# NJUVISION/PCGCv1

Hardware: AMD Instinct MI355X
Metric: 64³ cubes/sec encode+decode (hyper/a6b3); bpp & D1-PSNR vs reference (higher is better)
Workload: dtype f32; 1 GPU; synthetic longdress_vox10-like cloud (seed 1300, 1024^3): 828225 points -> 205 cubes of 64^3, --mode=hyper --cube_size=64 --min_num=64, the hyper/a6b3 checkpoint trained with this repository's train_hyper step on seeded synthetic surfaces (checkpoints/hyper/a6.00b3.00, tools/train_ckpt.py; the cloud was held out), compress_hyper + decompress_hyper incl. host range coding; cubes_per_rank=205, stream_crc32=2267905730

## Files before the change

### pcgcv1_amd/csrc/vrn_row16.hip

```cpp
#include "row_common.h"

namespace pcgc {

constexpr int kW16 = 16;
constexpr int kRowQ16 = kW16 * 16;

__device__ __forceinline__ float rshr1(float v) {
  return __builtin_bit_cast(float, __builtin_amdgcn_update_dpp(0, __builtin_bit_cast(int, v), 0x111, 0xf, 0xf, true));
}
__device__ __forceinline__ float rshl1(float v) {
  return __builtin_bit_cast(float, __builtin_amdgcn_update_dpp(0, __builtin_bit_cast(int, v), 0x101, 0xf, 0xf, true));
}

template <int NQ>
__device__ __forceinline__ f32x4 load_vec(i32x4 rs, int lane_off, int lane_row, int p, int q, int a) {
  const bool ok = (unsigned)p < (unsigned)kW16 && (unsigned)(a + lane_row) < (unsigned)kW16;
  const int base = ((p * kW16 + a) * NQ + q) * kRowQ16;
  return raw_load4(rs, ok ? base + lane_off : kOOB, 0, 0);
}

struct Tile16 {
  int b, k, d0;
};
template <int LD>
__device__ __forceinline__ Tile16 wave_tile16() {
  int wv = __builtin_amdgcn_readfirstlane(blockIdx.x * 8 + (threadIdx.x >> 6));
  Tile16 t;
  t.k = wv % 4; wv /= 4;
  t.d0 = (wv % (kW16 / LD)) * LD; wv /= (kW16 / LD);
  t.b = wv;
  return t;
}

constexpr int kVrn64ImgA = 16 * 28 * 64, kVrn64ImgB = 8 * 27 * 64, kVrn64ImgC = 4 * 27 * 64;
constexpr int kVrn64ImageFloats = kVrn64ImgA + kVrn64ImgB + kVrn64ImgC;

struct Vrn64Args {
  const float* img = nullptr;
  const float* x;
  float* t12;
  float* out;
  const float *w11, *b11, *w21, *b21, *w12, *b12, *w22, *b22, *w23, *b23;
  int B;
};

template <int NCO, int NC, int W2 = -1>
__device__ __forceinline__ void vec_channels(f32x4 (&acc)[3][NCO], f32x4* acc2, const float (&W)[28], int c0, const f32x4 (&X)[3], bool v0,
                                             bool v1, bool v2) {
  float x0[NC][3], xm[NC][3], xp[NC][3];
#pragma unroll
  for (int c = 0; c < NC; ++c)
#pragma unroll
    for (int kh = 0; kh < 3; ++kh) { x0[c][kh] = comp(X[kh], c0 + c); xm[c][kh] = rshr1(x0[c][kh]); xp[c][kh] = rshl1(x0[c][kh]); }
  const bool vj[3] = {v0, v1, v2};
#pragma unroll
  for (int jj = 0; jj < 3; ++jj) {
    const int kd = 2 - jj;
    if (vj[jj]) {
#pragma unroll
      for (int c = 0; c < NC; ++c) {
#pragma unroll
        for (int kh = 0; kh < 3; ++kh)
#pragma unroll
          for (int kw = 0; kw < 3; ++kw) {
            const int t = (kd * 3 + kh) * 3 + kw;
            const float xv = kw == 0 ? xm[c][kh] : (kw == 1 ? x0[c][kh] : xp[c][kh]);
#pragma unroll
            for (int coq = 0; coq < NCO; ++coq) acc[jj][coq] = mfa((c0 + c) * 4 + coq, W[t], xv, acc[jj][coq]);
          }
        if constexpr (W2 >= 0) {
          if (jj == 1) {
#pragma unroll
            for (int coq = 0; coq < NCO; ++coq) acc2[coq] = mfa((c0 + c) * 4 + coq, W[W2], x0[c][1], acc2[coq]);
          }
        }
      }
    }
  }
}

constexpr int kA64Chunk = 28 * 64;

template <int LD, bool = true>
__global__ void __launch_bounds__(512, 2) vrn64a_row_kernel(Vrn64Args a) {
  constexpr int CH = kA64Chunk;
  __shared__ float wl[16 * CH];
  if (a.img) stage_image_t<16 * CH, 512>(wl, a.img);
  else
    for (int i = threadIdx.x; i < 16 * CH; i += 512) {
      const int q = i / CH, f = i - q * CH;
      wl[i] = f < 1728 ? a.w11[((f >> 6) * 64 + 4 * q + ((f >> 4) & 3)) * 16 + (f & 15)] : a.w21[(4 * q + ((f - 1728) >> 4)) * 16 + (f & 15)];
    }
  __syncthreads();
  const int lane = threadIdx.x & 63;
  const int lane_row = lane >> 4;
  const Tile16 tl = wave_tile16<LD>();
  if (tl.b >= a.B) return;
  const int r0 = 4 * tl.k, d0 = tl.d0;
  f32x4 bi[4], bi2[4];
#pragma unroll
  for (int q = 0; q < 4; ++q) {
    bi[q] = f32x4{a.b11[4 * q], a.b11[4 * q + 1], a.b11[4 * q + 2], a.b11[4 * q + 3]};
    bi2[q] = f32x4{a.b21[4 * q], a.b21[4 * q + 1], a.b21[4 * q + 2], a.b21[4 * q + 3]};
  }
  f32x4 acc[3][4], acc2[4];
#pragma unroll
  for (int j = 0; j < 3; ++j)
#pragma unroll
    for (int q = 0; q < 4; ++q) acc[j][q] = bi[q];
  const i32x4 rs = make_rsrc(a.x + (size_t)tl.b * kW16 * kW16 * kW16 * 64, kW16 * kW16 * kW16 * 64 * 4);
  const int lane_off = lane_row * (16 * kRowQ16) + (lane & 15) * 16;
  f32x4* tb = reinterpret_cast<f32x4*>(a.t12) + (size_t)tl.b * kW16 * kW16 * 8 * kW16 + lane_row * (8 * kW16) + (lane & 15);
  f32x4 XA[3], XB[3];
  auto load = [&](f32x4 (&X)[3], int p, int q) {
#pragma unroll
    for (int kh = 0; kh < 3; ++kh) X[kh] = load_vec<16>(rs, lane_off, lane_row, p, q, r0 + kh - 1);
  };
  auto fetch = [&](float (&W)[28], int q) {
#pragma unroll
    for (int v = 0; v < 28; ++v) W[v] = wl[q * CH + v * 64 + lane];
  };
  auto quad = [&](const f32x4 (&X)[3], const float (&W)[28], bool v0, bool v1, bool v2) {
    vec_channels<4, 4, 27>(acc, acc2, W, 0, X, v0, v1, v2);
  };
  float WA[28], WB[28];
  load(XA, d0 - 1, 0);
  fetch(WA, 0);
#pragma unroll 1
  for (int p = d0 - 1; p <= d0 + LD; ++p) {
    const bool pin = (unsigned)p < (unsigned)kW16;
    const bool v0 = pin && p - 1 >= d0, v1 = pin && p >= d0 && p < d0 + LD, v2 = pin && p + 1 < d0 + LD;
#pragma unroll
    for (int q = 0; q < 4; ++q) acc2[q] = bi2[q];
#pragma unroll 1
    for (int q = 0; q < 16; q += 2) {
      load(XB, p, q + 1);
      fetch(WB, q + 1);
      quad(XA, WA, v0, v1, v2);
      if (q + 2 < 16) load(XA, p, q + 2); else load(XA, p + 1, 0);
      fetch(WA, (q + 2) & 15);
      quad(XB, WB, v0, v1, v2);
    }
    if (v1) {
#pragma unroll
      for (int coq = 0; coq < 4; ++coq) tb[((size_t)(p * kW16 + r0) * 8 + 4 + coq) * kW16] = relu4(acc2[coq]);
    }
    if (p - 1 >= d0) {
#pragma unroll
      for (int coq = 0; coq < 4; ++coq) tb[((size_t)((p - 1) * kW16 + r0) * 8 + coq) * kW16] = relu4(acc[0][coq]);
    }
#pragma unroll
    for (int coq = 0; coq < 4; ++coq) { acc[0][coq] = acc[1][coq]; acc[1][coq] = acc[2][coq]; acc[2][coq] = bi[coq]; }
  }
}

template <int LD, bool = true>
__global__ void __launch_bounds__(512, 2) vrn64b_row_kernel(Vrn64Args a) {
  constexpr int CH = 27 * 64;
  __shared__ float wl[8 * CH];
  if (a.img) stage_image_t<8 * CH, 512>(wl, a.img + kVrn64ImgA);
  else
    for (int i = threadIdx.x; i < 8 * CH; i += 512) {
      const int qh = i / CH, f = i - qh * CH, q = qh >> 1, half = qh & 1;
      wl[i] = a.w12[((f >> 6) * 16 + 4 * q + ((f >> 4) & 3)) * 32 + 16 * half + (f & 15)];
    }
  __syncthreads();
  const int lane = threadIdx.x & 63;
  const int lane_row = lane >> 4;
  const Tile16 tl = wave_tile16<LD>();
  if (tl.b >= a.B) return;
  const int r0 = 4 * tl.k, d0 = tl.d0;
  f32x4 bi[8];
#pragma unroll
  for (int q = 0; q < 8; ++q) bi[q] = f32x4{a.b12[4 * q], a.b12[4 * q + 1], a.b12[4 * q + 2], a.b12[4 * q + 3]};
  f32x4 accL[3][4], accH[3][4];
#pragma unroll
  for (int j = 0; j < 3; ++j)
#pragma unroll
    for (int q = 0; q < 4; ++q) { accL[j][q] = bi[q]; accH[j][q] = bi[4 + q]; }
  const i32x4 rs = make_rsrc(a.t12 + (size_t)tl.b * kW16 * kW16 * kW16 * 32, kW16 * kW16 * kW16 * 32 * 4);
  const i32x4 rx = make_rsrc(a.x + (size_t)tl.b * kW16 * kW16 * kW16 * 64, kW16 * kW16 * kW16 * 64 * 4);
  const i32x4 ro = make_rsrc(a.out + (size_t)tl.b * kW16 * kW16 * kW16 * 64, kW16 * kW16 * kW16 * 64 * 4);
  const int lane_off = lane_row * (8 * kRowQ16) + (lane & 15) * 16;
  const int lane_off_x = lane_row * (16 * kRowQ16) + (lane & 15) * 16;
  f32x4 XA[3], XB[3];
  auto load = [&](f32x4 (&X)[3], int p, int q) {
#pragma unroll
    for (int kh = 0; kh < 3; ++kh) X[kh] = load_vec<8>(rs, lane_off, lane_row, p, q, r0 + kh - 1);
  };
  auto quad = [&](const f32x4 (&X)[3], int q, bool v0, bool v1, bool v2) {
    float W[28];
#pragma unroll
    for (int v = 0; v < 27; ++v) W[v] = wl[(2 * q) * CH + v * 64 + lane];
    vec_channels<4, 4>(accL, nullptr, W, 0, X, v0, v1, v2);
#pragma unroll
    for (int v = 0; v < 27; ++v) W[v] = wl[(2 * q + 1) * CH + v * 64 + lane];
    vec_channels<4, 4>(accH, nullptr, W, 0, X, v0, v1, v2);
  };
  load(XA, d0 - 1, 0);
#pragma unroll 1
  for (int p = d0 - 1; p <= d0 + LD; ++p) {
    const bool pin = (unsigned)p < (unsigned)kW16;
    const bool v0 = pin && p - 1 >= d0, v1 = pin && p >= d0 && p < d0 + LD, v2 = pin && p + 1 < d0 + LD;
    load(XB, p, 1);
    quad(XA, 0, v0, v1, v2);
    load(XA, p, 2);
    const int obase = p - 1 >= d0 ? ((p - 1) * kW16 + r0) * (16 * kRowQ16) + lane_off_x : kOOB;
    f32x4 res[8];
#pragma unroll
    for (int q = 0; q < 8; ++q) res[q] = raw_load4(rx, obase + q * kRowQ16, 0, 0);
    quad(XB, 1, v0, v1, v2);
    load(XB, p, 3);
    quad(XA, 2, v0, v1, v2);
    load(XA, p + 1, 0);
    quad(XB, 3, v0, v1, v2);
#pragma unroll
    for (int q = 0; q < 4; ++q) {
      raw_store4(relu4(res[q] + relu4(accL[0][q])), ro, obase + q * kRowQ16, 0, 0);
      raw_store4(relu4(res[4 + q] + relu4(accH[0][q])), ro, obase + (4 + q) * kRowQ16, 0, 0);
    }
#pragma unroll
    for (int q = 0; q < 4; ++q) {
      accL[0][q] = accL[1][q]; accL[1][q] = accL[2][q]; accL[2][q] = bi[q];
      accH[0][q] = accH[1][q]; accH[1][q] = accH[2][q]; accH[2][q] = bi[4 + q];
    }
  }
}

template <int LD, bool = false>
__global__ void __launch_bounds__(512, 2) vrn64c_row_kernel(Vrn64Args a) {
  constexpr int CH = 27 * 64;
  __shared__ float wl[4 * CH];
  if (a.img) stage_image_t<4 * CH, 512>(wl, a.img + kVrn64ImgA + kVrn64ImgB);
  else
    for (int i = threadIdx.x; i < 4 * CH; i += 512) {
      const int q = i / CH, f = i - q * CH;
      wl[i] = a.w22[((f >> 6) * 16 + 4 * q + ((f >> 4) & 3)) * 16 + (f & 15)];
    }
  __syncthreads();
  const int lane = threadIdx.x & 63;
  const int lane_row = lane >> 4;
  const Tile16 tl = wave_tile16<LD>();
  if (tl.b >= a.B) return;
  const int r0 = 4 * tl.k, d0 = tl.d0;
  float W23[8];
#pragma unroll
  for (int v = 0; v < 8; ++v) W23[v] = a.w23[v * 64 + lane];
  f32x4 bi22[4], bi23[8];
#pragma unroll
  for (int q = 0; q < 4; ++q) bi22[q] = f32x4{a.b22[4 * q], a.b22[4 * q + 1], a.b22[4 * q + 2], a.b22[4 * q + 3]};
#pragma unroll
  for (int q = 0; q < 8; ++q) bi23[q] = f32x4{a.b23[4 * q], a.b23[4 * q + 1], a.b23[4 * q + 2], a.b23[4 * q + 3]};
  f32x4 acc[3][4];
#pragma unroll
  for (int j = 0; j < 3; ++j)
#pragma unroll
    for (int q = 0; q < 4; ++q) acc[j][q] = bi22[q];
  const i32x4 rs = make_rsrc(a.t12 + (size_t)tl.b * kW16 * kW16 * kW16 * 32, kW16 * kW16 * kW16 * 32 * 4);
  const i32x4 rx = make_rsrc(a.x + (size_t)tl.b * kW16 * kW16 * kW16 * 64, kW16 * kW16 * kW16 * 64 * 4);
  const i32x4 ro = make_rsrc(a.out + (size_t)tl.b * kW16 * kW16 * kW16 * 64, kW16 * kW16 * kW16 * 64 * 4);
  const int lane_off = lane_row * (8 * kRowQ16) + (lane & 15) * 16;
  const int lane_off_x = lane_row * (16 * kRowQ16) + (lane & 15) * 16;
  f32x4 XA[3], XB[3];
  auto load = [&](f32x4 (&X)[3], int p, int q) {
#pragma unroll
    for (int kh = 0; kh < 3; ++kh) X[kh] = load_vec<8>(rs, lane_off, lane_row, p, 4 + q, r0 + kh - 1);
  };
  auto quad = [&](const f32x4 (&X)[3], int q, bool v0, bool v1, bool v2) {
    float W[28];
#pragma unroll
    for (int v = 0; v < 27; ++v) W[v] = wl[q * CH + v * 64 + lane];
#pragma unroll
    for (int c = 0; c < 4; ++c) vec_channels<4, 1>(acc, nullptr, W, c, X, v0, v1, v2);
  };
  load(XA, d0 - 1, 0);
#pragma unroll 1
  for (int p = d0 - 1; p <= d0 + LD; ++p) {
    const bool pin = (unsigned)p < (unsigned)kW16;
    const bool v0 = pin && p - 1 >= d0, v1 = pin && p >= d0 && p < d0 + LD, v2 = pin && p + 1 < d0 + LD;
    load(XB, p, 1);
    quad(XA, 0, v0, v1, v2);
    load(XA, p, 2);
    const int obase = p - 1 >= d0 ? ((p - 1) * kW16 + r0) * (16 * kRowQ16) + 8 * kRowQ16 + lane_off_x : kOOB;
    f32x4 res[8];
#pragma unroll
    for (int q = 0; q < 8; ++q) res[q] = raw_load4(rx, obase + q * kRowQ16, 0, 0);
    quad(XB, 1, v0, v1, v2);
    load(XB, p, 3);
    quad(XA, 2, v0, v1, v2);
    load(XA, p + 1, 0);
    quad(XB, 3, v0, v1, v2);
    f32x4 t22[4], q3[8];
#pragma unroll
    for (int q = 0; q < 4; ++q) t22[q] = relu4(acc[0][q]);
#pragma unroll
    for (int q = 0; q < 8; ++q) q3[q] = bi23[q];
#pragma unroll
    for (int ci = 0; ci < 16; ++ci)
#pragma unroll
      for (int coq = 0; coq < 8; ++coq) q3[coq] = mfa((ci & 1) * 8 + coq, W23[ci >> 1], comp(t22[ci >> 2], ci & 3), q3[coq]);
#pragma unroll
    for (int q = 0; q < 8; ++q) raw_store4(relu4(res[q] + relu4(q3[q])), ro, obase + q * kRowQ16, 0, 0);
#pragma unroll
    for (int q = 0; q < 4; ++q) { acc[0][q] = acc[1][q]; acc[1][q] = acc[2][q]; acc[2][q] = bi22[q]; }
  }
}

struct Up1Args {
  const float* x;
  float* y;
  const float* w;
  const float* bias;
  int B, relu;
};
constexpr int kUp1Group = 16 * 27 * 32;

template <int LD>
__global__ void __launch_bounds__(256, 2) up1_row_kernel(Up1Args a) {
  constexpr int NCO = 2, CHT = 16 * NCO, CH = 27 * CHT, NW = (CH + 63) / 64;
  __shared__ __attribute__((aligned(16))) float wl[kUp1Group + 64];
  int wg = blockIdx.x;
  const int g = wg & 3; wg >>= 2;
  stage_image<kUp1Group>(wl, a.w + (size_t)g * kUp1Group);
  if (threadIdx.x < 64) wl[kUp1Group + threadIdx.x] = 0.f;
  __syncthreads();
  const int lane = threadIdx.x & 63, lane_row = lane >> 4;
  const int k = threadIdx.x >> 6;
  const int d0 = (wg % (kW16 / LD)) * LD;
  const int b = wg / (kW16 / LD);
  if (b >= a.B) return;
  f32x4 bi[NCO];
#pragma unroll
  for (int c = 0; c < NCO; ++c) {
    bi[c] = f32x4{0.f, 0.f, 0.f, 0.f};
    if (a.bias) bi[c] = f32x4{a.bias[(g * NCO + c) * 4], a.bias[(g * NCO + c) * 4 + 1], a.bias[(g * NCO + c) * 4 + 2], a.bias[(g * NCO + c) * 4 + 3]};
  }
  f32x4 acc[3][2][2][NCO];
#pragma unroll
  for (int s_ = 0; s_ < 3; ++s_)
#pragma unroll
    for (int ph = 0; ph < 2; ++ph)
#pragma unroll
      for (int pw = 0; pw < 2; ++pw)
#pragma unroll
        for (int c = 0; c < NCO; ++c) acc[s_][ph][pw][c] = bi[c];
  const i32x4 rs = make_rsrc(a.x + (size_t)b * kW16 * kW16 * kW16 * 64, kW16 * kW16 * kW16 * 64 * 4);
  const i32x4 ro = make_rsrc(a.y + (size_t)b * 32 * 32 * 32 * 32, 32 * 32 * 32 * 32 * 4);
  const int lane_off = lane_row * (16 * kRowQ16) + (lane & 15) * 16;
  const int out_lane = ((8 * k + 2 * lane_row) * 8 + g * NCO) * 512 + (lane & 15) * 32;
  f32x4 PA, OA, PB, OB;
  auto load = [&](f32x4& P, f32x4& O, int p, int q) {
    P = load_vec<16>(rs, lane_off, lane_row, p, q, 4 * k);
    O = load_vec<16>(rs, lane_off, lane_row, p, q, 4 * k - 1);
  };
  auto quad = [&](const f32x4& P, const f32x4& O, int q, bool v0, bool v2) {
    float W[NW];
#pragma unroll
    for (int v = 0; v < NW; ++v) W[v] = wl[q * CH + v * 64 + lane];
#pragma unroll
    for (int c = 0; c < 4; ++c) {
      const float x0 = comp(P, c), x1 = comp(O, c);
      const float r0 = rshr1(x0), r1 = rshr1(x1);
      const bool vj[3] = {v0, v0, v2};
#pragma unroll
      for (int s_ = 0; s_ < 3; ++s_) {
        if (vj[s_]) {
#pragma unroll
          for (int co = 0; co < NCO; ++co) {
            auto mf_ = [&](int kh, int kw, float xv, f32x4& d) {
              const int t = (s_ * 3 + kh) * 3 + kw, fo = t * CHT + c * 4 * NCO + co * 4;
              d = mfa((fo & 63) >> 2, W[fo >> 6], xv, d);
            };
            mf_(0, 0, x0, acc[s_][0][0][co]); mf_(0, 2, r0, acc[s_][0][0][co]); mf_(2, 0, x1, acc[s_][0][0][co]); mf_(2, 2, r1, acc[s_][0][0][co]);
            mf_(0, 1, x0, acc[s_][0][1][co]); mf_(2, 1, x1, acc[s_][0][1][co]);
            mf_(1, 0, x0, acc[s_][1][0][co]); mf_(1, 2, r0, acc[s_][1][0][co]);
            mf_(1, 1, x0, acc[s_][1][1][co]);
          }
        }
      }
    }
  };
  auto store_plane = [&](int set, int od, bool ok) {
    const int base = ok ? od * (32 * 8 * 512) + out_lane : kOOB;
#pragma unroll
    for (int ph = 0; ph < 2; ++ph)
#pragma unroll
      for (int co = 0; co < NCO; ++co)
#pragma unroll
        for (int pw = 0; pw < 2; ++pw) {
          f32x4 v = acc[set][ph][pw][co];
          if (a.relu) v = relu4(v);
          raw_store4(v, ro, base + (ph * 8 + co) * 512 + pw * 16, 0, 0);
        }
  };
  load(PA, OA, d0 - 1, 0);
#pragma unroll 1
  for (int p = d0 - 1; p < d0 + LD; ++p) {
    const bool v0 = p >= d0, v2 = p >= 0 && p + 1 < d0 + LD;
#pragma unroll 1
    for (int q = 0; q < 16; q += 2) {
      load(PB, OB, p, q + 1);
      quad(PA, OA, q, v0, v2);
      if (q + 2 < 16) load(PA, OA, p, q + 2); else load(PA, OA, p + 1, 0);
      quad(PB, OB, q + 1, v0, v2);
    }
    store_plane(0, 2 * p, v0);
    store_plane(1, 2 * p + 1, v0);
#pragma unroll
    for (int ph = 0; ph < 2; ++ph)
#pragma unroll
      for (int pw = 0; pw < 2; ++pw)
#pragma unroll
        for (int c = 0; c < NCO; ++c) { acc[0][ph][pw][c] = acc[2][ph][pw][c]; acc[1][ph][pw][c] = bi[c]; acc[2][ph][pw][c] = bi[c]; }
  }
}

__global__ void __launch_bounds__(256) up1_image_kernel(const float* w, float* dst) {
  const int i = blockIdx.x * 256 + threadIdx.x;
  if (i >= 4 * kUp1Group) return;
  const int g = i / kUp1Group, f0 = i - g * kUp1Group, q = f0 / 864, f = f0 - q * 864;
  const int tap = f >> 5, c = (f >> 3) & 3, co = f & 7;
  dst[i] = w[(tap * 32 + g * 8 + co) * 64 + 4 * q + c];
}
size_t up1_image_floats() { return 4 * (size_t)kUp1Group; }
int launch_up1_image(const float* w_tf, float* dst, hipStream_t s) {
  hipLaunchKernelGGL(up1_image_kernel, dim3((4 * kUp1Group + 255) / 256), dim3(256), 0, s, w_tf, dst);
  return launch_ok("up1_image_kernel");
}
int launch_up1_row(const float* x, float* y, const float* w_image, const float* bias, int B, int relu, hipStream_t s) {
  Up1Args a{x, y, w_image, bias, B, relu};
  constexpr int LD = 4;
  hipLaunchKernelGGL((up1_row_kernel<LD>), dim3(B * (kW16 / LD) * 4), dim3(256), 0, s, a);
  return launch_ok("up1_row_kernel");
}

constexpr int kDown2Group = 8 * 27 * 128;

template <int LD>
__global__ void __launch_bounds__(512, 2) down2_row_kernel(Up1Args a) {
  constexpr int NCO = 8, CHT = 16 * NCO, CH = 27 * CHT, NWK = 9 * CHT / 64;
  __shared__ __attribute__((aligned(16))) float wl[kDown2Group];
  int wg = blockIdx.x;
  const int g = wg & 1; wg >>= 1;
  for (int i = threadIdx.x * 4; i < kDown2Group; i += 2048)
    *reinterpret_cast<float4*>(&wl[i]) = *reinterpret_cast<const float4*>(&a.w[(size_t)g * kDown2Group + i]);
  __syncthreads();
  const int lane = threadIdx.x & 63, lane_row = lane >> 4, wave = threadIdx.x >> 6;
  const int k = wave & 3;
  constexpr int SEGS = kW16 / LD;
  const int seg = (wg % (SEGS / 2)) * 2 + (wave >> 2);
  const int b = wg / (SEGS / 2);
  const int d0 = seg * LD;
  if (b >= a.B) return;
  f32x4 bi[NCO];
#pragma unroll
  for (int c = 0; c < NCO; ++c) {
    bi[c] = f32x4{0.f, 0.f, 0.f, 0.f};
    if (a.bias) bi[c] = f32x4{a.bias[(g * NCO + c) * 4], a.bias[(g * NCO + c) * 4 + 1], a.bias[(g * NCO + c) * 4 + 2], a.bias[(g * NCO + c) * 4 + 3]};
  }
  f32x4 cur[NCO], nxt[NCO];
#pragma unroll
  for (int c = 0; c < NCO; ++c) { cur[c] = bi[c]; nxt[c] = bi[c]; }
  const i32x4 rs = make_rsrc(a.x + (size_t)b * 32 * 32 * 32 * 32, 32 * 32 * 32 * 32 * 4);
  const i32x4 ro = make_rsrc(a.y + (size_t)b * kW16 * kW16 * kW16 * 64, kW16 * kW16 * kW16 * 64 * 4);
  const int in_lane = lane_row * (2 * 8 * 512) + (lane & 15) * 32;
  const int out_lane = ((4 * k + lane_row) * 16 + g * NCO) * kRowQ16 + (lane & 15) * 16;
  struct Rows { f32x4 e[3], o[3]; };
  auto load = [&](Rows& R, int p, int q) {
#pragma unroll
    for (int kh = 0; kh < 3; ++kh) {
      const int ih = 8 * k + kh;
      const bool ok = (unsigned)p < 32u && ih + 2 * lane_row < 32;
      const int off = ok ? ((p * 32 + ih) * 8 + q) * 512 + in_lane : kOOB;
      R.e[kh] = raw_load4(rs, off, 0, 0);
      R.o[kh] = raw_load4(rs, off + 16, 0, 0);
    }
  };
  auto quad = [&](const Rows& R, int q, int KA, f32x4 (&accA)[NCO], int KB, f32x4 (&accB)[NCO], bool vB) {
#pragma unroll
    for (int pass = 0; pass < 2; ++pass) {
      const int kd = pass == 0 ? KA : KB;
      if (kd < 0 || (pass == 1 && !vB)) continue;
      float W[NWK];
#pragma unroll
      for (int vv = 0; vv < NWK; ++vv) W[vv] = wl[q * CH + kd * 9 * CHT + vv * 64 + lane];
      f32x4 (&acc)[NCO] = pass == 0 ? accA : accB;
#pragma unroll
      for (int c = 0; c < 4; ++c)
#pragma unroll
        for (int kh = 0; kh < 3; ++kh) {
          const float xe = comp(R.e[kh], c), xo = comp(R.o[kh], c), x2 = rshl1(xe);
#pragma unroll
          for (int kw = 0; kw < 3; ++kw) {
            const float xv = kw == 0 ? xe : (kw == 1 ? xo : x2);
#pragma unroll
            for (int co = 0; co < NCO; ++co) {
              const int fo = (kh * 3 + kw) * CHT + c * 4 * NCO + co * 4;
              acc[co] = mfa((fo & 63) >> 2, W[fo >> 6], xv, acc[co]);
            }
          }
        }
    }
  };
  Rows RA, RB;
  load(RA, 2 * d0, 0);
#pragma unroll 1
  for (int q = 0; q < 8; ++q) {
    if (q + 1 < 8) load(RB, 2 * d0, q + 1); else load(RB, 2 * d0 + 1, 0);
    quad(RA, q, 0, cur, -1, nxt, false);
    RA = RB;
  }
#pragma unroll 1
  for (int j = d0; j < d0 + LD; ++j) {
#pragma unroll 1
    for (int q = 0; q < 8; ++q) {
      if (q + 1 < 8) load(RB, 2 * j + 1, q + 1); else load(RB, 2 * j + 2, 0);
      quad(RA, q, 1, cur, -1, nxt, false);
      RA = RB;
    }
    const bool more = j + 1 < d0 + LD;
#pragma unroll 1
    for (int q = 0; q < 8; ++q) {
      if (q + 1 < 8) load(RB, 2 * j + 2, q + 1); else load(RB, 2 * j + 3, 0);
      quad(RA, q, 2, cur, 0, nxt, more);
      RA = RB;
    }
#pragma unroll
    for (int co = 0; co < NCO; ++co) {
      f32x4 v = cur[co];
      if (a.relu) v = relu4(v);
      raw_store4(v, ro, j * (kW16 * 16 * kRowQ16) + out_lane + co * kRowQ16, 0, 0);
      cur[co] = nxt[co];
      nxt[co] = bi[co];
    }
  }
}

__global__ void __launch_bounds__(256) down2_image_kernel(const float* w, float* dst) {
  const int i = blockIdx.x * 256 + threadIdx.x;
  if (i >= 2 * kDown2Group) return;
  const int g = i / kDown2Group, f0 = i - g * kDown2Group, q = f0 / 3456, f = f0 - q * 3456;
  const int tap = f >> 7, c = (f >> 5) & 3, co = f & 31;
  dst[i] = w[(tap * 32 + 4 * q + c) * 64 + g * 32 + co];
}
size_t down2_image_floats() { return 2 * (size_t)kDown2Group; }
int launch_down2_image(const float* w_tf, float* dst, hipStream_t s) {
  hipLaunchKernelGGL(down2_image_kernel, dim3((2 * kDown2Group + 255) / 256), dim3(256), 0, s, w_tf, dst);
  return launch_ok("down2_image_kernel");
}
int launch_down2_row(const float* x, float* y, const float* w_image, const float* bias, int B, int relu, hipStream_t s) {
  Up1Args a{x, y, w_image, bias, B, relu};
  const char* e = getenv("PCGC_DOWN2_LD");
  int ld = e ? atoi(e) : 0;
  if (ld != 1 && ld != 2 && ld != 4) {
    double best = 1e30;
    for (int c : {4, 2, 1}) {
      const int wgs = B * 16 / c, rounds = (wgs + 255) / 256;
      const double cost = (1.0 + 0.125 / c) * rounds * 256.0 / wgs;
      if (cost < best - 1e-9) { best = cost; ld = c; }
    }
  }
  if (ld == 1) hipLaunchKernelGGL((down2_row_kernel<1>), dim3(B * (kW16 / 1 / 2) * 2), dim3(512), 0, s, a);
  else if (ld == 4) hipLaunchKernelGGL((down2_row_kernel<4>), dim3(B * (kW16 / 4 / 2) * 2), dim3(512), 0, s, a);
  else hipLaunchKernelGGL((down2_row_kernel<2>), dim3(B * (kW16 / 2 / 2) * 2), dim3(512), 0, s, a);
  return launch_ok("down2_row_kernel");
}

__global__ void __launch_bounds__(256) vrn64_image_kernel(const float* w11, const float* w21, const float* w12, const float* w22, float* dst) {
  const int i = blockIdx.x * 256 + threadIdx.x;
  if (i >= kVrn64ImageFloats) return;
  if (i < kVrn64ImgA) {
    constexpr int CH = 28 * 64;
    const int q = i / CH, f = i - q * CH;
    dst[i] = f < 1728 ? w11[((f >> 6) * 64 + 4 * q + ((f >> 4) & 3)) * 16 + (f & 15)] : w21[(4 * q + ((f - 1728) >> 4)) * 16 + (f & 15)];
  } else if (i < kVrn64ImgA + kVrn64ImgB) {
    constexpr int CH = 27 * 64;
    const int j = i - kVrn64ImgA, qh = j / CH, f = j - qh * CH, q = qh >> 1, half = qh & 1;
    dst[i] = w12[((f >> 6) * 16 + 4 * q + ((f >> 4) & 3)) * 32 + 16 * half + (f & 15)];
  } else {
    constexpr int CH = 27 * 64;
    const int j = i - kVrn64ImgA - kVrn64ImgB, q = j / CH, f = j - q * CH;
    dst[i] = w22[((f >> 6) * 16 + 4 * q + ((f >> 4) & 3)) * 16 + (f & 15)];
  }
}
size_t vrn64_image_floats() { return kVrn64ImageFloats; }
int launch_vrn64_image(const float* const* w, float* dst, hipStream_t s) {
  hipLaunchKernelGGL(vrn64_image_kernel, dim3((kVrn64ImageFloats + 255) / 256), dim3(256), 0, s, w[0], w[4], w[2], w[6], dst);
  return launch_ok("vrn64_image_kernel");
}

int launch_vrn64_row(const float* x, float* t12, float* out, const float* const* w, int B, int which, hipStream_t s, const float* img) {
  Vrn64Args a;
  a.img = img;
  a.x = x; a.t12 = t12; a.out = out;
  a.w11 = w[0]; a.b11 = w[1]; a.w12 = w[2]; a.b12 = w[3]; a.w21 = w[4]; a.b21 = w[5];
  a.w22 = w[6]; a.b22 = w[7]; a.w23 = w[8]; a.b23 = w[9];
  a.B = B;
  const char* e_ld = getenv("PCGC_V64_LD");
  int ld = e_ld ? atoi(e_ld) : -1;
  if (ld == 0) ld = B * 16 < 512 ? 1 : (B * 16 < 2048 ? 2 : 4);
  if (ld != 1 && ld != 2 && ld != 4) {
    double best = 1e30;
    for (int c : {4, 2, 1}) {
      const int waves = B * 4 * (kW16 / c), rounds = (waves + 2047) / 2048;
      const double cost = (1.0 + 0.25 / c) * rounds * 2048.0 / waves;
      if (cost < best - 1e-9) { best = cost; ld = c; }
    }
  }
  if (ld == 1) {
    constexpr int LD = 1;
    const int blocks = (B * 4 * (kW16 / LD) + 7) / 8;
    if (which == 0) hipLaunchKernelGGL((vrn64a_row_kernel<LD>), dim3(blocks), dim3(512), 0, s, a);
    else if (which == 1) hipLaunchKernelGGL((vrn64b_row_kernel<LD>), dim3(blocks), dim3(512), 0, s, a);
    else hipLaunchKernelGGL((vrn64c_row_kernel<LD>), dim3(blocks), dim3(512), 0, s, a);
    return launch_ok("vrn64 row kernel");
  }
  if (ld == 2) {
    constexpr int LD = 2;
    const int blocks = (B * 4 * (kW16 / LD) + 7) / 8;
    if (which == 0) hipLaunchKernelGGL((vrn64a_row_kernel<LD>), dim3(blocks), dim3(512), 0, s, a);
    else if (which == 1) hipLaunchKernelGGL((vrn64b_row_kernel<LD>), dim3(blocks), dim3(512), 0, s, a);
    else hipLaunchKernelGGL((vrn64c_row_kernel<LD>), dim3(blocks), dim3(512), 0, s, a);
    return launch_ok("vrn64 row kernel");
  }
  constexpr int LD = 4;
  const int waves = B * 4 * (kW16 / LD);
  const int blocks = (waves + 7) / 8;
  if (which == 0) hipLaunchKernelGGL((vrn64a_row_kernel<LD>), dim3(blocks), dim3(512), 0, s, a);
  else if (which == 1) hipLaunchKernelGGL((vrn64b_row_kernel<LD>), dim3(blocks), dim3(512), 0, s, a);
  else hipLaunchKernelGGL((vrn64c_row_kernel<LD>), dim3(blocks), dim3(512), 0, s, a);
  return launch_ok("vrn64 row kernel");
}

}
```

Measured before the change: 5336 cubes/s.

## Balance vrn64 row-kernel work across a fixed wave budget with output-channel splits

Replaces the fixed depth-tile-per-wave mapping in the three vrn64 row kernels with a balanced split. Each wave now takes a contiguous share of (batch, row-group, channel-part, plane) units, possibly spanning two column pieces. For the a and b kernels, output channels can also be split across 2 or 4 waves (H parts), and a host cost model picks H. The aim is to cut tail imbalance when B*64 waves do not fill 2048 slots evenly, at the price of redundant halo planes and input loads per piece plus a few extra template variants.

Measured after the change: 5295 cubes/s. No clear change (-0.8%).

```diff
diff --git a/pcgcv1_amd/csrc/v64_split.h b/pcgcv1_amd/csrc/v64_split.h
--- /dev/null
+++ b/pcgcv1_amd/csrc/v64_split.h
@@ -0,0 +1,78 @@
+#pragma once
+
+#if defined(__HIPCC__)
+#define PCGC_V64_HD __host__ __device__ inline
+#else
+#define PCGC_V64_HD inline
+#endif
+
+namespace pcgc {
+
+constexpr int kV64Planes = 16;
+constexpr int kV64Shares = 2048;
+constexpr int kV64MaxShare = 17;
+
+struct V64Split {
+  int waves;
+  int base, rem;
+  int hshift;
+  int ld;
+};
+struct V64Piece {
+  int b, k, h, d0, len;
+};
+
+PCGC_V64_HD int v64_units(int B, int H) { return B * 4 * H * kV64Planes; }
+PCGC_V64_HD int v64_largest_share(int B, int H, int shares = kV64Shares) {
+  const int U = v64_units(B, H), S = U < shares ? U : shares;
+  return S > 0 ? (U + S - 1) / S : 0;
+}
+PCGC_V64_HD bool v64_balanced_ok(int B, int H, int shares = kV64Shares) { return B > 0 && v64_largest_share(B, H, shares) <= kV64MaxShare; }
+
+PCGC_V64_HD V64Split v64_split(int B, int H, int ld, int shares = kV64Shares) {
+  V64Split s;
+  s.hshift = H == 4 ? 2 : (H == 2 ? 1 : 0);
+  s.ld = ld;
+  if (ld) {
+    s.hshift = 0;
+    s.waves = B * 4 * (kV64Planes / ld);
+    s.base = ld;
+    s.rem = 0;
+  } else {
+    const int U = v64_units(B, H);
+    s.waves = U < shares ? U : shares;
+    s.base = s.waves > 0 ? U / s.waves : 0;
+    s.rem = s.waves > 0 ? U % s.waves : 0;
+  }
+  return s;
+}
+
+PCGC_V64_HD V64Piece v64_piece(const V64Split& s, int w, int i) {
+  V64Piece p{0, 0, 0, 0, 0};
+  if (w < 0 || w >= s.waves) return p;
+  int col, d0, n;
+  if (s.ld) {
+    if (i) return p;
+    const int tshift = s.ld == 4 ? 2 : (s.ld == 2 ? 3 : 4);
+    const int k = w & 3, bt = w >> 2;
+    col = (bt >> tshift) * 4 + k;
+    d0 = (bt & ((1 << tshift) - 1)) * s.ld;
+    n = s.ld;
+  } else {
+    const int u = w * s.base + (w < s.rem ? w : s.rem);
+    n = s.base + (w < s.rem ? 1 : 0);
+    col = u / kV64Planes;
+    d0 = u % kV64Planes;
+    const int first = n < kV64Planes - d0 ? n : kV64Planes - d0;
+    if (i) { col += 1; d0 = 0; n -= first; }
+    else n = first;
+  }
+  p.h = col & ((1 << s.hshift) - 1);
+  p.k = (col >> s.hshift) & 3;
+  p.b = col >> (s.hshift + 2);
+  p.d0 = d0;
+  p.len = n;
+  return p;
+}
+
+}
diff --git a/pcgcv1_amd/csrc/vrn_row16.hip b/pcgcv1_amd/csrc/vrn_row16.hip
--- a/pcgcv1_amd/csrc/vrn_row16.hip
+++ b/pcgcv1_amd/csrc/vrn_row16.hip
@@ -1,4 +1,5 @@
 #include "row_common.h"
+#include "v64_split.h"
 
 namespace pcgc {
 
@@ -17,19 +18,6 @@
   const bool ok = (unsigned)p < (unsigned)kW16 && (unsigned)(a + lane_row) < (unsigned)kW16;
   const int base = ((p * kW16 + a) * NQ + q) * kRowQ16;
   return raw_load4(rs, ok ? base + lane_off : kOOB, 0, 0);
-}
-
-struct Tile16 {
-  int b, k, d0;
-};
-template <int LD>
-__device__ __forceinline__ Tile16 wave_tile16() {
-  int wv = __builtin_amdgcn_readfirstlane(blockIdx.x * 8 + (threadIdx.x >> 6));
-  Tile16 t;
-  t.k = wv % 4; wv /= 4;
-  t.d0 = (wv % (kW16 / LD)) * LD; wv /= (kW16 / LD);
-  t.b = wv;
-  return t;
 }
 
 constexpr int kVrn64ImgA = 16 * 28 * 64, kVrn64ImgB = 8 * 27 * 64, kVrn64ImgC = 4 * 27 * 64;
@@ -41,7 +29,7 @@
   float* t12;
   float* out;
   const float *w11, *b11, *w21, *b21, *w12, *b12, *w22, *b22, *w23, *b23;
-  int B;
+  V64Split sp;
 };
 
 template <int NCO, int NC, int W2 = -1>
@@ -79,9 +67,13 @@
   }
 }
 
+__device__ __forceinline__ int wave_index16() { return __builtin_amdgcn_readfirstlane(blockIdx.x * 8 + (threadIdx.x >> 6)); }
+__device__ __forceinline__ int part_lane(int lane, int coq0) { return (lane & ~12) | ((lane + 4 * coq0) & 12); }
+__device__ __forceinline__ f32x4 bias_quad(const float* b, int q) { return f32x4{b[4 * q], b[4 * q + 1], b[4 * q + 2], b[4 * q + 3]}; }
+
 constexpr int kA64Chunk = 28 * 64;
 
-template <int LD, bool = true>
+template <int NCO>
 __global__ void __launch_bounds__(512, 2) vrn64a_row_kernel(Vrn64Args a) {
   constexpr int CH = kA64Chunk;
   __shared__ float wl[16 * CH];
@@ -94,67 +86,70 @@
   __syncthreads();
   const int lane = threadIdx.x & 63;
   const int lane_row = lane >> 4;
-  const Tile16 tl = wave_tile16<LD>();
-  if (tl.b >= a.B) return;
-  const int r0 = 4 * tl.k, d0 = tl.d0;
-  f32x4 bi[4], bi2[4];
-#pragma unroll
-  for (int q = 0; q < 4; ++q) {
-    bi[q] = f32x4{a.b11[4 * q], a.b11[4 * q + 1], a.b11[4 * q + 2], a.b11[4 * q + 3]};
-    bi2[q] = f32x4{a.b21[4 * q], a.b21[4 * q + 1], a.b21[4 * q + 2], a.b21[4 * q + 3]};
-  }
-  f32x4 acc[3][4], acc2[4];
-#pragma unroll
-  for (int j = 0; j < 3; ++j)
-#pragma unroll
-    for (int q = 0; q < 4; ++q) acc[j][q] = bi[q];
-  const i32x4 rs = make_rsrc(a.x + (size_t)tl.b * kW16 * kW16 * kW16 * 64, kW16 * kW16 * kW16 * 64 * 4);
-  const int lane_off = lane_row * (16 * kRowQ16) + (lane & 15) * 16;
-  f32x4* tb = reinterpret_cast<f32x4*>(a.t12) + (size_t)tl.b * kW16 * kW16 * 8 * kW16 + lane_row * (8 * kW16) + (lane & 15);
-  f32x4 XA[3], XB[3];
-  auto load = [&](f32x4 (&X)[3], int p, int q) {
-#pragma unroll
-    for (int kh = 0; kh < 3; ++kh) X[kh] = load_vec<16>(rs, lane_off, lane_row, p, q, r0 + kh - 1);
-  };
-  auto fetch = [&](float (&W)[28], int q) {
-#pragma unroll
-    for (int v = 0; v < 28; ++v) W[v] = wl[q * CH + v * 64 + lane];
-  };
-  auto quad = [&](const f32x4 (&X)[3], const float (&W)[28], bool v0, bool v1, bool v2) {
-    vec_channels<4, 4, 27>(acc, acc2, W, 0, X, v0, v1, v2);
-  };
-  float WA[28], WB[28];
-  load(XA, d0 - 1, 0);
-  fetch(WA, 0);
-#pragma unroll 1
-  for (int p = d0 - 1; p <= d0 + LD; ++p) {
-    const bool pin = (unsigned)p < (unsigned)kW16;
-    const bool v0 = pin && p - 1 >= d0, v1 = pin && p >= d0 && p < d0 + LD, v2 = pin && p + 1 < d0 + LD;
-#pragma unroll
-    for (int q = 0; q < 4; ++q) acc2[q] = bi2[q];
-#pragma unroll 1
-    for (int q = 0; q < 16; q += 2) {
-      load(XB, p, q + 1);
-      fetch(WB, q + 1);
-      quad(XA, WA, v0, v1, v2);
-      if (q + 2 < 16) load(XA, p, q + 2); else load(XA, p + 1, 0);
-      fetch(WA, (q + 2) & 15);
-      quad(XB, WB, v0, v1, v2);
-    }
-    if (v1) {
-#pragma unroll
-      for (int coq = 0; coq < 4; ++coq) tb[((size_t)(p * kW16 + r0) * 8 + 4 + coq) * kW16] = relu4(acc2[coq]);
-    }
-    if (p - 1 >= d0) {
-#pragma unroll
-      for (int coq = 0; coq < 4; ++coq) tb[((size_t)((p - 1) * kW16 + r0) * 8 + coq) * kW16] = relu4(acc[0][coq]);
-    }
-#pragma unroll
-    for (int coq = 0; coq < 4; ++coq) { acc[0][coq] = acc[1][coq]; acc[1][coq] = acc[2][coq]; acc[2][coq] = bi[coq]; }
-  }
-}
-
-template <int LD, bool = true>
+  const int wv = wave_index16();
+#pragma unroll 1
+  for (int piece = 0; piece < 2; ++piece) {
+    const V64Piece pc = v64_piece(a.sp, wv, piece);
+    if (pc.len == 0) break;
+    const int r0 = 4 * pc.k, d0 = pc.d0, d1 = pc.d0 + pc.len, coq0 = pc.h * NCO;
+    int wlane = part_lane(lane, coq0);
+    f32x4 bi[NCO], bi2[NCO];
+#pragma unroll
+    for (int q = 0; q < NCO; ++q) { bi[q] = bias_quad(a.b11, coq0 + q); bi2[q] = bias_quad(a.b21, coq0 + q); }
+    f32x4 acc[3][NCO], acc2[NCO];
+#pragma unroll
+    for (int j = 0; j < 3; ++j)
+#pragma unroll
+      for (int q = 0; q < NCO; ++q) acc[j][q] = bi[q];
+    const i32x4 rs = make_rsrc(a.x + (size_t)pc.b * kW16 * kW16 * kW16 * 64, kW16 * kW16 * kW16 * 64 * 4);
+    const int lane_off = lane_row * (16 * kRowQ16) + (lane & 15) * 16;
+    f32x4* tb = reinterpret_cast<f32x4*>(a.t12) + (size_t)pc.b * kW16 * kW16 * 8 * kW16 + lane_row * (8 * kW16) + (lane & 15) + coq0 * kW16;
+    f32x4 XA[3], XB[3];
+    auto load = [&](f32x4 (&X)[3], int p, int q) {
+#pragma unroll
+      for (int kh = 0; kh < 3; ++kh) X[kh] = load_vec<16>(rs, lane_off, lane_row, p, q, r0 + kh - 1);
+    };
+    auto fetch = [&](float (&W)[28], int q) {
+#pragma unroll
+      for (int v = 0; v < 28; ++v) W[v] = wl[q * CH + v * 64 + wlane];
+    };
+    auto quad = [&](const f32x4 (&X)[3], const float (&W)[28], bool v0, bool v1, bool v2) {
+      vec_channels<NCO, 4, 27>(acc, acc2, W, 0, X, v0, v1, v2);
+    };
+    float WA[28], WB[28];
+    load(XA, d0 - 1, 0);
+    fetch(WA, 0);
+#pragma unroll 1
+    for (int p = d0 - 1; p <= d1; ++p) {
+      const bool pin = (unsigned)p < (unsigned)kW16;
+      asm volatile("" : "+v"(wlane));
+      const bool v0 = pin && p - 1 >= d0, v1 = pin && p >= d0 && p < d1, v2 = pin && p + 1 < d1;
+#pragma unroll
+      for (int q = 0; q < NCO; ++q) acc2[q] = bi2[q];
+#pragma unroll 1
+      for (int q = 0; q < 16; q += 2) {
+        load(XB, p, q + 1);
+        fetch(WB, q + 1);
+        quad(XA, WA, v0, v1, v2);
+        if (q + 2 < 16) load(XA, p, q + 2); else load(XA, p + 1, 0);
+        fetch(WA, (q + 2) & 15);
+        quad(XB, WB, v0, v1, v2);
+      }
+      if (v1) {
+#pragma unroll
+        for (int coq = 0; coq < NCO; ++coq) tb[((size_t)(p * kW16 + r0) * 8 + 4 + coq) * kW16] = relu4(acc2[coq]);
+      }
+      if (p - 1 >= d0) {
+#pragma unroll
+        for (int coq = 0; coq < NCO; ++coq) tb[((size_t)((p - 1) * kW16 + r0) * 8 + coq) * kW16] = relu4(acc[0][coq]);
+      }
+#pragma unroll
+      for (int coq = 0; coq < NCO; ++coq) { acc[0][coq] = acc[1][coq]; acc[1][coq] = acc[2][coq]; acc[2][coq] = bi[coq]; }
+    }
+  }
+}
+
+template <int NH, int NQ>
 __global__ void __launch_bounds__(512, 2) vrn64b_row_kernel(Vrn64Args a) {
   constexpr int CH = 27 * 64;
   __shared__ float wl[8 * CH];
@@ -167,67 +162,78 @@
   __syncthreads();
   const int lane = threadIdx.x & 63;
   const int lane_row = lane >> 4;
-  const Tile16 tl = wave_tile16<LD>();
-  if (tl.b >= a.B) return;
-  const int r0 = 4 * tl.k, d0 = tl.d0;
-  f32x4 bi[8];
-#pragma unroll
-  for (int q = 0; q < 8; ++q) bi[q] = f32x4{a.b12[4 * q], a.b12[4 * q + 1], a.b12[4 * q + 2], a.b12[4 * q + 3]};
-  f32x4 accL[3][4], accH[3][4];
-#pragma unroll
-  for (int j = 0; j < 3; ++j)
-#pragma unroll
-    for (int q = 0; q < 4; ++q) { accL[j][q] = bi[q]; accH[j][q] = bi[4 + q]; }
-  const i32x4 rs = make_rsrc(a.t12 + (size_t)tl.b * kW16 * kW16 * kW16 * 32, kW16 * kW16 * kW16 * 32 * 4);
-  const i32x4 rx = make_rsrc(a.x + (size_t)tl.b * kW16 * kW16 * kW16 * 64, kW16 * kW16 * kW16 * 64 * 4);
-  const i32x4 ro = make_rsrc(a.out + (size_t)tl.b * kW16 * kW16 * kW16 * 64, kW16 * kW16 * kW16 * 64 * 4);
-  const int lane_off = lane_row * (8 * kRowQ16) + (lane & 15) * 16;
-  const int lane_off_x = lane_row * (16 * kRowQ16) + (lane & 15) * 16;
-  f32x4 XA[3], XB[3];
-  auto load = [&](f32x4 (&X)[3], int p, int q) {
-#pragma unroll
-    for (int kh = 0; kh < 3; ++kh) X[kh] = load_vec<8>(rs, lane_off, lane_row, p, q, r0 + kh - 1);
-  };
-  auto quad = [&](const f32x4 (&X)[3], int q, bool v0, bool v1, bool v2) {
-    float W[28];
-#pragma unroll
-    for (int v = 0; v < 27; ++v) W[v] = wl[(2 * q) * CH + v * 64 + lane];
-    vec_channels<4, 4>(accL, nullptr, W, 0, X, v0, v1, v2);
-#pragma unroll
-    for (int v = 0; v < 27; ++v) W[v] = wl[(2 * q + 1) * CH + v * 64 + lane];
-    vec_channels<4, 4>(accH, nullptr, W, 0, X, v0, v1, v2);
-  };
-  load(XA, d0 - 1, 0);
-#pragma unroll 1
-  for (int p = d0 - 1; p <= d0 + LD; ++p) {
-    const bool pin = (unsigned)p < (unsigned)kW16;
-    const bool v0 = pin && p - 1 >= d0, v1 = pin && p >= d0 && p < d0 + LD, v2 = pin && p + 1 < d0 + LD;
-    load(XB, p, 1);
-    quad(XA, 0, v0, v1, v2);
-    load(XA, p, 2);
-    const int obase = p - 1 >= d0 ? ((p - 1) * kW16 + r0) * (16 * kRowQ16) + lane_off_x : kOOB;
-    f32x4 res[8];
-#pragma unroll
-    for (int q = 0; q < 8; ++q) res[q] = raw_load4(rx, obase + q * kRowQ16, 0, 0);
-    quad(XB, 1, v0, v1, v2);
-    load(XB, p, 3);
-    quad(XA, 2, v0, v1, v2);
-    load(XA, p + 1, 0);
-    quad(XB, 3, v0, v1, v2);
-#pragma unroll
-    for (int q = 0; q < 4; ++q) {
-      raw_store4(relu4(res[q] + relu4(accL[0][q])), ro, obase + q * kRowQ16, 0, 0);
-      raw_store4(relu4(res[4 + q] + relu4(accH[0][q])), ro, obase + (4 + q) * kRowQ16, 0, 0);
-    }
-#pragma unroll
-    for (int q = 0; q < 4; ++q) {
-      accL[0][q] = accL[1][q]; accL[1][q] = accL[2][q]; accL[2][q] = bi[q];
-      accH[0][q] = accH[1][q]; accH[1][q] = accH[2][q]; accH[2][q] = bi[4 + q];
-    }
-  }
-}
-
-template <int LD, bool = false>
+  const int wv = wave_index16();
+#pragma unroll 1
+  for (int piece = 0; piece < 2; ++piece) {
+    const V64Piece pc = v64_piece(a.sp, wv, piece);
+    if (pc.len == 0) break;
+    const int r0 = 4 * pc.k, d0 = pc.d0, d1 = pc.d0 + pc.len;
+    const int half0 = NH == 2 ? 0 : (NQ == 2 ? pc.h >> 1 : pc.h), coq0 = NQ == 2 ? (pc.h & 1) * 2 : 0;
+    const int oq0 = half0 * 4 + coq0;
+    int wlane = part_lane(lane, coq0);
+    f32x4 bi[NH][NQ];
+#pragma unroll
+    for (int hf = 0; hf < NH; ++hf)
+#pragma unroll
+      for (int q = 0; q < NQ; ++q) bi[hf][q] = bias_quad(a.b12, oq0 + 4 * hf + q);
+    f32x4 acc[NH][3][NQ];
+#pragma unroll
+    for (int hf = 0; hf < NH; ++hf)
+#pragma unroll
+      for (int j = 0; j < 3; ++j)
+#pragma unroll
+        for (int q = 0; q < NQ; ++q) acc[hf][j][q] = bi[hf][q];
+    const i32x4 rs = make_rsrc(a.t12 + (size_t)pc.b * kW16 * kW16 * kW16 * 32, kW16 * kW16 * kW16 * 32 * 4);
+    const i32x4 rx = make_rsrc(a.x + (size_t)pc.b * kW16 * kW16 * kW16 * 64, kW16 * kW16 * kW16 * 64 * 4);
+    const i32x4 ro = make_rsrc(a.out + (size_t)pc.b * kW16 * kW16 * kW16 * 64, kW16 * kW16 * kW16 * 64 * 4);
+    const int lane_off = lane_row * (8 * kRowQ16) + (lane & 15) * 16;
+    const int lane_off_x = lane_row * (16 * kRowQ16) + (lane & 15) * 16 + oq0 * kRowQ16;
+    f32x4 XA[3], XB[3];
+    auto load = [&](f32x4 (&X)[3], int p, int q) {
+#pragma unroll
+      for (int kh = 0; kh < 3; ++kh) X[kh] = load_vec<8>(rs, lane_off, lane_row, p, q, r0 + kh - 1);
+    };
+    auto quad = [&](const f32x4 (&X)[3], int q, bool v0, bool v1, bool v2) {
+      float W[28];
+#pragma unroll
+      for (int hf = 0; hf < NH; ++hf) {
+#pragma unroll
+        for (int v = 0; v < 27; ++v) W[v] = wl[(2 * q + half0 + hf) * CH + v * 64 + wlane];
+        vec_channels<NQ, 4>(acc[hf], nullptr, W, 0, X, v0, v1, v2);
+      }
+    };
+    load(XA, d0 - 1, 0);
+#pragma unroll 1
+    for (int p = d0 - 1; p <= d1; ++p) {
+      const bool pin = (unsigned)p < (unsigned)kW16;
+      asm volatile("" : "+v"(wlane));
+      const bool v0 = pin && p - 1 >= d0, v1 = pin && p >= d0 && p < d1, v2 = pin && p + 1 < d1;
+      load(XB, p, 1);
+      quad(XA, 0, v0, v1, v2);
+      load(XA, p, 2);
+      const int obase = p - 1 >= d0 ? ((p - 1) * kW16 + r0) * (16 * kRowQ16) + lane_off_x : kOOB;
+      f32x4 res[NH][NQ];
+#pragma unroll
+      for (int hf = 0; hf < NH; ++hf)
+#pragma unroll
+        for (int q = 0; q < NQ; ++q) res[hf][q] = raw_load4(rx, obase + (4 * hf + q) * kRowQ16, 0, 0);
+      quad(XB, 1, v0, v1, v2);
+      load(XB, p, 3);
+      quad(XA, 2, v0, v1, v2);
+      load(XA, p + 1, 0);
+      quad(XB, 3, v0, v1, v2);
+#pragma unroll
+      for (int q = 0; q < NQ; ++q)
+#pragma unroll
+        for (int hf = 0; hf < NH; ++hf) raw_store4(relu4(res[hf][q] + relu4(acc[hf][0][q])), ro, obase + (4 * hf + q) * kRowQ16, 0, 0);
+#pragma unroll
+      for (int hf = 0; hf < NH; ++hf)
+#pragma unroll
+        for (int q = 0; q < NQ; ++q) { acc[hf][0][q] = acc[hf][1][q]; acc[hf][1][q] = acc[hf][2][q]; acc[hf][2][q] = bi[hf][q]; }
+    }
+  }
+}
+
 __global__ void __launch_bounds__(512, 2) vrn64c_row_kernel(Vrn64Args a) {
   constexpr int CH = 27 * 64;
   __shared__ float wl[4 * CH];
@@ -240,69 +246,75 @@
   __syncthreads();
   const int lane = threadIdx.x & 63;
   const int lane_row = lane >> 4;
-  const Tile16 tl = wave_tile16<LD>();
-  if (tl.b >= a.B) return;
-  const int r0 = 4 * tl.k, d0 = tl.d0;
-  float W23[8];
-#pragma unroll
-  for (int v = 0; v < 8; ++v) W23[v] = a.w23[v * 64 + lane];
-  f32x4 bi22[4], bi23[8];
-#pragma unroll
-  for (int q = 0; q < 4; ++q) bi22[q] = f32x4{a.b22[4 * q], a.b22[4 * q + 1], a.b22[4 * q + 2], a.b22[4 * q + 3]};
-#pragma unroll
-  for (int q = 0; q < 8; ++q) bi23[q] = f32x4{a.b23[4 * q], a.b23[4 * q + 1], a.b23[4 * q + 2], a.b23[4 * q + 3]};
-  f32x4 acc[3][4];
-#pragma unroll
-  for (int j = 0; j < 3; ++j)
-#pragma unroll
-    for (int q = 0; q < 4; ++q) acc[j][q] = bi22[q];
-  const i32x4 rs = make_rsrc(a.t12 + (size_t)tl.b * kW16 * kW16 * kW16 * 32, kW16 * kW16 * kW16 * 32 * 4);
-  const i32x4 rx = make_rsrc(a.x + (size_t)tl.b * kW16 * kW16 * kW16 * 64, kW16 * kW16 * kW16 * 64 * 4);
-  const i32x4 ro = make_rsrc(a.out + (size_t)tl.b * kW16 * kW16 * kW16 * 64, kW16 * kW16 * kW16 * 64 * 4);
-  const int lane_off = lane_row * (8 * kRowQ16) + (lane & 15) * 16;
-  const int lane_off_x = lane_row * (16 * kRowQ16) + (lane & 15) * 16;
-  f32x4 XA[3], XB[3];
-  auto load = [&](f32x4 (&X)[3], int p, int q) {
-#pragma unroll
-    for (int kh = 0; kh < 3; ++kh) X[kh] = load_vec<8>(rs, lane_off, lane_row, p, 4 + q, r0 + kh - 1);
-  };
-  auto quad = [&](const f32x4 (&X)[3], int q, bool v0, bool v1, bool v2) {
-    float W[28];
-#pragma unroll
-    for (int v = 0; v < 27; ++v) W[v] = wl[q * CH + v * 64 + lane];
-#pragma unroll
-    for (int c = 0; c < 4; ++c) vec_channels<4, 1>(acc, nullptr, W, c, X, v0, v1, v2);
-  };
-  load(XA, d0 - 1, 0);
-#pragma unroll 1
-  for (int p = d0 - 1; p <= d0 + LD; ++p) {
-    const bool pin = (unsigned)p < (unsigned)kW16;
-    const bool v0 = pin && p - 1 >= d0, v1 = pin && p >= d0 && p < d0 + LD, v2 = pin && p + 1 < d0 + LD;
-    load(XB, p, 1);
-    quad(XA, 0, v0, v1, v2);
-    load(XA, p, 2);
-    const int obase = p - 1 >= d0 ? ((p - 1) * kW16 + r0) * (16 * kRowQ16) + 8 * kRowQ16 + lane_off_x : kOOB;
-    f32x4 res[8];
-#pragma unroll
-    for (int q = 0; q < 8; ++q) res[q] = raw_load4(rx, obase + q * kRowQ16, 0, 0);
-    quad(XB, 1, v0, v1, v2);
-    load(XB, p, 3);
-    quad(XA, 2, v0, v1, v2);
-    load(XA, p + 1, 0);
-    quad(XB, 3, v0, v1, v2);
-    f32x4 t22[4], q3[8];
-#pragma unroll
-    for (int q = 0; q < 4; ++q) t22[q] = relu4(acc[0][q]);
-#pragma unroll
-    for (int q = 0; q < 8; ++q) q3[q] = bi23[q];
-#pragma unroll
-    for (int ci = 0; ci < 16; ++ci)
-#pragma unroll
-      for (int coq = 0; coq < 8; ++coq) q3[coq] = mfa((ci & 1) * 8 + coq, W23[ci >> 1], comp(t22[ci >> 2], ci & 3), q3[coq]);
-#pragma unroll
-    for (int q = 0; q < 8; ++q) raw_store4(relu4(res[q] + relu4(q3[q])), ro, obase + q * kRowQ16, 0, 0);
-#pragma unroll
-    for (int q = 0; q < 4; ++q) { acc[0][q] = acc[1][q]; acc[1][q] = acc[2][q]; acc[2][q] = bi22[q]; }
+  const int wv = wave_index16();
+#pragma unroll 1
+  for (int piece = 0; piece < 2; ++piece) {
+    const V64Piece pc = v64_piece(a.sp, wv, piece);
+    if (pc.len == 0) break;
+    const int r0 = 4 * pc.k, d0 = pc.d0, d1 = pc.d0 + pc.len;
+    int wlane = lane;
+    float W23[8];
+#pragma unroll
+    for (int v = 0; v < 8; ++v) W23[v] = a.w23[v * 64 + lane];
+    f32x4 bi22[4], bi23[8];
+#pragma unroll
+    for (int q = 0; q < 4; ++q) bi22[q] = bias_quad(a.b22, q);
+#pragma unroll
+    for (int q = 0; q < 8; ++q) bi23[q] = bias_quad(a.b23, q);
+    f32x4 acc[3][4];
+#pragma unroll
+    for (int j = 0; j < 3; ++j)
+#pragma unroll
+      for (int q = 0; q < 4; ++q) acc[j][q] = bi22[q];
+    const i32x4 rs = make_rsrc(a.t12 + (size_t)pc.b * kW16 * kW16 * kW16 * 32, kW16 * kW16 * kW16 * 32 * 4);
+    const i32x4 rx = make_rsrc(a.x + (size_t)pc.b * kW16 * kW16 * kW16 * 64, kW16 * kW16 * kW16 * 64 * 4);
+    const i32x4 ro = make_rsrc(a.out + (size_t)pc.b * kW16 * kW16 * kW16 * 64, kW16 * kW16 * kW16 * 64 * 4);
+    const int lane_off = lane_row * (8 * kRowQ16) + (lane & 15) * 16;
+    const int lane_off_x = lane_row * (16 * kRowQ16) + (lane & 15) * 16;
+    f32x4 XA[3], XB[3];
+    auto load = [&](f32x4 (&X)[3], int p, int q) {
+#pragma unroll
+      for (int kh = 0; kh < 3; ++kh) X[kh] = load_vec<8>(rs, lane_off, lane_row, p, 4 + q, r0 + kh - 1);
+    };
+    auto quad = [&](const f32x4 (&X)[3], int q, bool v0, bool v1, bool v2) {
+      float W[28];
+#pragma unroll
+      for (int v = 0; v < 27; ++v) W[v] = wl[q * CH + v * 64 + wlane];
+#pragma unroll
+      for (int c = 0; c < 4; ++c) vec_channels<4, 1>(acc, nullptr, W, c, X, v0, v1, v2);
+    };
+    load(XA, d0 - 1, 0);
+#pragma unroll 1
+    for (int p = d0 - 1; p <= d1; ++p) {
+      const bool pin = (unsigned)p < (unsigned)kW16;
+      asm volatile("" : "+v"(wlane));
+      const bool v0 = pin && p - 1 >= d0, v1 = pin && p >= d0 && p < d1, v2 = pin && p + 1 < d1;
+      load(XB, p, 1);
+      quad(XA, 0, v0, v1, v2);
+      load(XA, p, 2);
+      const int obase = p - 1 >= d0 ? ((p - 1) * kW16 + r0) * (16 * kRowQ16) + 8 * kRowQ16 + lane_off_x : kOOB;
+      f32x4 res[8];
+#pragma unroll
+      for (int q = 0; q < 8; ++q) res[q] = raw_load4(rx, obase + q * kRowQ16, 0, 0);
+      quad(XB, 1, v0, v1, v2);
+      load(XB, p, 3);
+      quad(XA, 2, v0, v1, v2);
+      load(XA, p + 1, 0);
+      quad(XB, 3, v0, v1, v2);
+      f32x4 t22[4], q3[8];
+#pragma unroll
+      for (int q = 0; q < 4; ++q) t22[q] = relu4(acc[0][q]);
+#pragma unroll
+      for (int q = 0; q < 8; ++q) q3[q] = bi23[q];
+#pragma unroll
+      for (int ci = 0; ci < 16; ++ci)
+#pragma unroll
+        for (int coq = 0; coq < 8; ++coq) q3[coq] = mfa((ci & 1) * 8 + coq, W23[ci >> 1], comp(t22[ci >> 2], ci & 3), q3[coq]);
+#pragma unroll
+      for (int q = 0; q < 8; ++q) raw_store4(relu4(res[q] + relu4(q3[q])), ro, obase + q * kRowQ16, 0, 0);
+#pragma unroll
+      for (int q = 0; q < 4; ++q) { acc[0][q] = acc[1][q]; acc[1][q] = acc[2][q]; acc[2][q] = bi22[q]; }
+    }
   }
 }
 
@@ -589,46 +601,55 @@
   return launch_ok("vrn64_image_kernel");
 }
 
+constexpr double kV64PartCost[3] = {0.11, 0.03, 0.20};
+constexpr int kV64MaxParts[3] = {2, 4, 1};
+
+static int v64_balanced_parts(int B, int which) {
+  int H = 1;
+  double best = 1e30;
+  for (int h = 1; h <= kV64MaxParts[which]; h *= 2) {
+    if (!v64_balanced_ok(B, h)) continue;
+    const int n = v64_largest_share(B, h);
+    const double cost = (n + 2) * kV64PartCost[which] + (double)n / h;
+    if (cost < best - 1e-9) { best = cost; H = h; }
+  }
+  return H;
+}
+static int v64_fixed_tile(int B) {
+  int ld = 4;
+  double best = 1e30;
+  for (int c : {4, 2, 1}) {
+    const int waves = B * 4 * (kW16 / c), rounds = (waves + kV64Shares - 1) / kV64Shares;
+    const double cost = (1.0 + 0.25 / c) * rounds * (double)kV64Shares / waves;
+    if (cost < best - 1e-9) { best = cost; ld = c; }
+  }
+  return ld;
+}
+
 int launch_vrn64_row(const float* x, float* t12, float* out, const float* const* w, int B, int which, hipStream_t s, const float* img) {
   Vrn64Args a;
   a.img = img;
   a.x = x; a.t12 = t12; a.out = out;
   a.w11 = w[0]; a.b11 = w[1]; a.w12 = w[2]; a.b12 = w[3]; a.w21 = w[4]; a.b21 = w[5];
   a.w22 = w[6]; a.b22 = w[7]; a.w23 = w[8]; a.b23 = w[9];
-  a.B = B;
   const char* e_ld = getenv("PCGC_V64_LD");
-  int ld = e_ld ? atoi(e_ld) : -1;
+  const char* e_h = getenv("PCGC_V64_H");
+  int ld = e_ld ? atoi(e_ld) : -1, H = 1;
   if (ld == 0) ld = B * 16 < 512 ? 1 : (B * 16 < 2048 ? 2 : 4);
   if (ld != 1 && ld != 2 && ld != 4) {
-    double best = 1e30;
-    for (int c : {4, 2, 1}) {
-      const int waves = B * 4 * (kW16 / c), rounds = (waves + 2047) / 2048;
-      const double cost = (1.0 + 0.25 / c) * rounds * 2048.0 / waves;
-      if (cost < best - 1e-9) { best = cost; ld = c; }
-    }
-  }
-  if (ld == 1) {
-    constexpr int LD = 1;
-    const int blocks = (B * 4 * (kW16 / LD) + 7) / 8;
-    if (which == 0) hipLaunchKernelGGL((vrn64a_row_kernel<LD>), dim3(blocks), dim3(512), 0, s, a);
-    else if (which == 1) hipLaunchKernelGGL((vrn64b_row_kernel<LD>), dim3(blocks), dim3(512), 0, s, a);
-    else hipLaunchKernelGGL((vrn64c_row_kernel<LD>), dim3(blocks), dim3(512), 0, s, a);
-    return launch_ok("vrn64 row kernel");
-  }
-  if (ld == 2) {
-    constexpr int LD = 2;
-    const int blocks = (B * 4 * (kW16 / LD) + 7) / 8;
-    if (which == 0) hipLaunchKernelGGL((vrn64a_row_kernel<LD>), dim3(blocks), dim3(512), 0, s, a);
-    else if (which == 1) hipLaunchKernelGGL((vrn64b_row_kernel<LD>), dim3(blocks), dim3(512), 0, s, a);
-    else hipLaunchKernelGGL((vrn64c_row_kernel<LD>), dim3(blocks), dim3(512), 0, s, a);
-    return launch_ok("vrn64 row kernel");
-  }
-  constexpr int LD = 4;
-  const int waves = B * 4 * (kW16 / LD);
-  const int blocks = (waves + 7) / 8;
-  if (which == 0) hipLaunchKernelGGL((vrn64a_row_kernel<LD>), dim3(blocks), dim3(512), 0, s, a);
-  else if (which == 1) hipLaunchKernelGGL((vrn64b_row_kernel<LD>), dim3(blocks), dim3(512), 0, s, a);
-  else hipLaunchKernelGGL((vrn64c_row_kernel<LD>), dim3(blocks), dim3(512), 0, s, a);
+    ld = 0;
+    const int fh = e_h ? atoi(e_h) : 0;
+    const bool forced = fh == 1 || fh == 2 || fh == 4;
+    H = forced ? (which == 2 ? 1 : fh) : v64_balanced_parts(B, which);
+    const int n = v64_largest_share(B, H);
+    if (!v64_balanced_ok(B, H)) { ld = v64_fixed_tile(B); H = 1; }
+    else if (!forced && H == 1 && (n == 1 || n == 2 || n == 4)) ld = n;
+  }
+  a.sp = v64_split(B, H, ld);
+  void (*kernel)(Vrn64Args) = which == 2 ? vrn64c_row_kernel
+                              : which == 1 ? (H == 4 ? vrn64b_row_kernel<1, 2> : (H == 2 ? vrn64b_row_kernel<1, 4> : vrn64b_row_kernel<2, 4>))
+                                           : (H == 4 ? vrn64a_row_kernel<1> : (H == 2 ? vrn64a_row_kernel<2> : vrn64a_row_kernel<4>));
+  hipLaunchKernelGGL(kernel, dim3((a.sp.waves + 7) / 8), dim3(512), 0, s, a);
   return launch_ok("vrn64 row kernel");
 }
 
```
